# debbiemarkslab/BEAR

Measured on AMD Instinct MI355X. Metric: k-mer contexts/sec (DM-marginal+grad h), k=13, higher is better.
Workload: dtype f64

## Files before the change

### bear_amd/csrc/kernels_plan.h

```cpp
#pragma once
#include "kernels_sorted.h"

#ifndef PLN_THREADS
#define PLN_THREADS 1024
#endif
#define PLN_WAVES (PLN_THREADS / 64)
#ifndef PLN_UNITS
#define PLN_UNITS 32
#endif
#define PLN_NI (PLN_UNITS * 64)
#ifndef PLN_NI_CUT
#define PLN_NI_CUT PLN_NI
#endif
#ifndef PLN_RMAX
#define PLN_RMAX 1664
#endif
#ifndef PLN_HCAP
#define PLN_HCAP 128
#endif
#define PLN_NBIG 4096
#define PLN_BLOCKS_PER_CU (1024 / PLN_THREADS)
#define PLN_QUAD 4
#define PLN_LIVE_STRIDE (PLN_RMAX + 8)
#define PLN_SENTINEL (PLN_RMAX * 5)
#ifndef PLN_NBUF
#define PLN_NBUF 2
#endif
#define PLN_BLOCK_MAX (64 + PLN_RMAX + PLN_NI * 2 + PLN_HCAP * (2 + 4 + 2 + 8))

struct pln_tile {
  uint64_t row0;
  uint32_t rows_items;
  uint32_t off16;
  uint32_t hc_hr;
  uint32_t blk16;
  uint64_t pad;
};
static_assert(sizeof(pln_tile) == 32, "tile descriptors are fetched with one s_load_dwordx8");
#ifndef PLN_CHUNK
#define PLN_CHUNK 128
#endif
#ifndef PLN_DMA_WAVES
#define PLN_DMA_WAVES 2
#endif
#ifndef PLN_PREFETCH_KIB
#define PLN_PREFETCH_KIB 24
#endif
#define PLN_DESC_CHUNK 32
#define PLN_DESC_PAD (2 * PLN_DESC_CHUNK)

struct pln_layout {
  uint32_t nrow, items, hoff, hcnt, hrow, hn, end;
};
__host__ __device__ inline pln_layout pln_block_layout(uint32_t rows, uint32_t n_light, uint32_t hc, uint32_t hr) {
  pln_layout L;
  L.nrow = 64u;
  L.items = L.nrow + ((rows + 15u) & ~15u);
  L.hoff = L.items + (((n_light + 63u) & ~63u) * 2u);
  L.hcnt = L.hoff + (((hc + 7u) & ~7u) * 2u);
  L.hrow = L.hcnt + (((hc + 3u) & ~3u) * 4u);
  L.hn = L.hrow + (((hr + 7u) & ~7u) * 2u);
  L.end = L.hn + (((hr + 1u) & ~1u) * 8u);
  return L;
}

struct pln_heavy_col {
  uint64_t off;
  uint64_t c;
};

struct pln_heavy_row {
  uint64_t row;
  double n;
};

__global__ __launch_bounds__(256) void plan_scan_kernel(const uint32_t *__restrict__ counts, uint64_t n_rows, int ncol,
                                                        uint8_t *__restrict__ quad_light,
                                                        unsigned long long *__restrict__ heavy_counts,
                                                        unsigned long long *__restrict__ hist) {
  __shared__ uint32_t s_heavy[3];
  __shared__ uint32_t s_hist[2 * SRT_NKEY];
  __shared__ uint32_t s_big[PLN_NBIG + 1];
  __shared__ unsigned long long s_total, s_cells;
  __shared__ uint32_t s_cmax;
  unsigned long long my_total = 0ull;
  uint32_t my_cells = 0u, my_cmax = 0u;
  if (threadIdx.x == 0) {
    s_total = s_cells = 0ull;
    s_cmax = 0u;
  }
  if (threadIdx.x < 3) s_heavy[threadIdx.x] = 0;
  if (threadIdx.x < 2 * SRT_NKEY) s_hist[threadIdx.x] = 0;
  for (uint32_t k = threadIdx.x; k <= PLN_NBIG; k += 256) s_big[k] = 0;
  __syncthreads();
  const uint64_t n_quads = (n_rows + PLN_QUAD - 1) / PLN_QUAD;
  for (uint64_t g = (uint64_t)blockIdx.x * 256 + threadIdx.x; g < n_quads; g += (uint64_t)gridDim.x * 256) {
    uint32_t light = 0, qhc = 0, qhr = 0;
    for (uint64_t r = PLN_QUAD * g; r < PLN_QUAD * g + PLN_QUAD && r < n_rows; ++r) {
      uint32_t nsat = 0, hcol = 0;
#pragma unroll
      for (int b = 0; b < 5; ++b) {
        const uint32_t c = counts[r * 5 + b];
        const uint32_t s = nsat + c;
        nsat = s < nsat ? 0xffffffffu : s;
        my_total += c;
        my_cells += c != 0u;
        my_cmax = c > my_cmax ? c : my_cmax;
        if (b < ncol) {
          light += (c != 0 && c <= SRT_CL);
          hcol += (c > SRT_CL);
        }
      }
      qhc += hcol;
      qhr += nsat > SRT_CL;
      if (hcol) atomicAdd(&s_heavy[0], hcol);
      if (nsat > SRT_CL) {
        atomicAdd(&s_heavy[1], 1u);
        if (nsat <= PLN_NBIG) atomicAdd(&s_big[nsat], 1u);
      } else if (nsat != 0) atomicAdd(&s_hist[nsat - 1], 1u);
      const uint32_t c4 = counts[r * 5 + 4];
      if (ncol == 4 && c4 > SRT_CL) atomicAdd(&s_heavy[2], 1u);
      else if (ncol == 4 && c4 != 0) atomicAdd(&s_hist[SRT_NKEY + c4 - 1], 1u);
    }
    quad_light[g] = (uint8_t)light;
    quad_light[n_quads + g] = (uint8_t)qhc;
    quad_light[2 * n_quads + g] = (uint8_t)qhr;
  }
  if (my_total) {
    atomicAdd(&s_total, my_total);
    atomicAdd(&s_cells, (unsigned long long)my_cells);
    atomicMax(&s_cmax, my_cmax);
  }
  __syncthreads();
  if (threadIdx.x == 0 && s_total) {
    atomicAdd(&heavy_counts[6], s_total);
    atomicAdd(&heavy_counts[7], s_cells);
    atomicMax(&heavy_counts[8], (unsigned long long)s_cmax);
  }
  if (threadIdx.x < 3 && s_heavy[threadIdx.x]) atomicAdd(&heavy_counts[threadIdx.x], (unsigned long long)s_heavy[threadIdx.x]);
  if (threadIdx.x < 2 * SRT_NKEY && s_hist[threadIdx.x]) atomicAdd(&hist[threadIdx.x], (unsigned long long)s_hist[threadIdx.x]);
  for (uint32_t k = threadIdx.x; k <= PLN_NBIG; k += 256)
    if (s_big[k]) atomicAdd(&hist[2 * SRT_NKEY + k], (unsigned long long)s_big[k]);
}

#define PLN_CUT_CHUNK_MAX 8192
static inline uint32_t plan_cut_chunk(uint64_t n_quads) { return n_quads <= 50000000ull ? 2048u : (uint32_t)PLN_CUT_CHUNK_MAX; }
#define PLN_CUT_SPAN (PLN_RMAX / PLN_QUAD)

__device__ __forceinline__ uint64_t plan_cut_one(const uint8_t *__restrict__ quad, uint64_t n_quads, uint64_t q0, uint32_t *items,
                                                 uint32_t *hcol, uint32_t *hrow) {
  uint32_t it = 0, hc = 0, hr = 0, rows = 0;
  uint64_t q = q0;
  while (q < n_quads && rows + PLN_QUAD <= PLN_RMAX && it + quad[q] <= PLN_NI_CUT) {
    it += quad[q];
    if (hcol) {
      hc += quad[n_quads + q];
      hr += quad[2 * n_quads + q];
    }
    rows += PLN_QUAD;
    ++q;
  }
  *items = it;
  if (hcol) {
    *hcol = hc;
    *hrow = hr;
  }
  return q;
}
__global__ __launch_bounds__(256) void plan_cut_step_kernel(const uint8_t *__restrict__ quad, uint64_t n_quads, uint64_t n_chunks,
                                                            uint32_t chunk, uint16_t *__restrict__ step) {
  const uint64_t k = (uint64_t)blockIdx.x * 256 + threadIdx.x;
  if (k >= n_chunks) return;
  const uint64_t q0 = k * chunk, q_end = q0 + chunk < n_quads ? q0 + chunk : n_quads;
  uint64_t r = q0;
  uint32_t items = 0;
  for (uint64_t q = q0; q < q_end; ++q) {
    if (r < q) {
      r = q;
      items = 0;
    }
    while (r < n_quads && (uint32_t)(r - q + 1) * PLN_QUAD <= PLN_RMAX && items + quad[r] <= PLN_NI_CUT) items += quad[r++];
    step[q] = (uint16_t)(r - q);
    items -= quad[q];
  }
}
__global__ __launch_bounds__(256) void plan_cut_walk_kernel(const uint16_t *__restrict__ step, uint64_t n_quads, uint64_t n_chunks,
                                                            uint32_t chunk, uint32_t *__restrict__ walk) {
  const uint64_t id = (uint64_t)blockIdx.x * 256 + threadIdx.x;
  if (id >= n_chunks * PLN_CUT_SPAN) return;
  const uint64_t k = id / PLN_CUT_SPAN, j = id - k * PLN_CUT_SPAN, end = (k + 1) * chunk;
  uint64_t q = k * chunk + j;
  uint32_t cnt = 0;
  while (q < end && q < n_quads) {
    q += step[q];
    ++cnt;
  }
  walk[id] = (uint32_t)(q >= end ? q - end : 0) | (cnt << 16);
}
static_assert(PLN_CUT_CHUNK_MAX < 65536 && PLN_CUT_SPAN < 65536 && PLN_CUT_SPAN <= 2048, "walk table: 16-bit fields; a tile is shorter than a chunk");
// ... 226 lines not shown
    if (tid == 31) E[31] = (uint16_t)hr_cap;
#pragma unroll
    for (int k = 0; k < RPT; ++k)
#pragma unroll
      for (int b = 0; b < 5; ++b)
        if (c[k][b] != 0) sorted[offs[(c[k][b] - 1) * SRT_REP + rep] + rank[k][b]] = (uint16_t)((tid + 1024u * k) * 5 + b);
    __syncthreads();
#ifdef BEAR_DET_BUILD
    {
      for (uint32_t i = tid; i < PLN_NI; i += 1024) {
        uint32_t key = 0;
        for (uint32_t q = 1; q < SRT_CL; ++q) key += offs[q * SRT_REP] <= i ? 1u : 0u;
        comp[i] = i < n_light ? (key << 16) | sorted[i] : 0xffffffffu;
      }
      __syncthreads();
      for (uint32_t size = 2; size <= PLN_NI; size <<= 1)
        for (uint32_t stride = size >> 1; stride > 0; stride >>= 1) {
          const uint32_t lo = 2u * tid - (tid & (stride - 1u)), hi = lo + stride;
          if (tid < PLN_NI / 2) {
            const bool up = (lo & size) == 0u;
            const uint32_t a = comp[lo], bq = comp[hi];
            if ((a > bq) == up) {
              comp[lo] = bq;
              comp[hi] = a;
            }
          }
          __syncthreads();
        }
      for (uint32_t i = tid; i < n_light; i += 1024) sorted[i] = (uint16_t)(comp[i] & 0xffffu);
      __syncthreads();
      const uint32_t nhc = s_hc < hc_cap ? s_hc : hc_cap, nhr = s_hr < hr_cap ? s_hr : hr_cap;
      if (tid < nhc) hkey[tid] = ((unsigned long long)hoff[tid] << 32) | hcnt[tid];
      __syncthreads();
      if (tid < nhc) {
        uint32_t r = 0;
        for (uint32_t q = 0; q < nhc; ++q) r += hkey[q] < hkey[tid] ? 1u : 0u;
        htmp[r] = hkey[tid];
      }
      __syncthreads();
      if (tid < nhc) {
        hoff[tid] = (uint16_t)(htmp[tid] >> 32);
        hcnt[tid] = (uint32_t)htmp[tid];
      }
      __syncthreads();
      if (tid < nhr) hkey[tid] = ((unsigned long long)hrow[tid] << 48) | tid;
      if (tid < nhr) htmp[tid] = (unsigned long long)__double_as_longlong(hn[tid]);
      __syncthreads();
      uint32_t r = 0;
      unsigned long long mine = 0ull, myn = 0ull;
      if (tid < nhr) {
        for (uint32_t q = 0; q < nhr; ++q) r += hkey[q] < hkey[tid] ? 1u : 0u;
        mine = hkey[tid];
        myn = htmp[tid];
      }
      __syncthreads();
      if (tid < nhr) {
        hrow[r] = (uint16_t)(mine >> 48);
        hn[r] = __longlong_as_double((long long)myn);
      }
      __syncthreads();
    }
#endif
    const uint32_t padded = (n_light + 63u) & ~63u;
    for (uint32_t i = tid; i < padded; i += 1024) items[i] = i < n_light ? sorted[i] : (uint16_t)PLN_SENTINEL;
    __syncthreads();
  }
}

__global__ __launch_bounds__(1024) void plan_live_kernel(const pln_tile *__restrict__ tiles, uint64_t n_tiles,
                                                         const unsigned char *__restrict__ stream, uint16_t *__restrict__ live) {
  constexpr int RPT = (PLN_RMAX + 1023) / 1024;
  __shared__ uint32_t cnt[RPT * 16];
  const uint32_t tid = threadIdx.x, lane = tid & 63, wave = tid >> 6;
  for (uint64_t t = blockIdx.x; t < n_tiles; t += gridDim.x) {
    const pln_tile ti = tiles[t];
    const uint32_t rows = ti.rows_items >> 16;
    const uint8_t *nrow = stream + (size_t)ti.off16 * 16 + 64;
    uint16_t *out = live + t * PLN_LIVE_STRIDE;
    unsigned long long mask[RPT];
#pragma unroll
    for (int k = 0; k < RPT; ++k) {
      const uint32_t lr = tid + 1024u * k;
      mask[k] = __builtin_amdgcn_ballot_w64(lr < rows && nrow[lr] != 0);
      if (lane == 0) cnt[k * 16 + wave] = (uint32_t)__builtin_popcountll(mask[k]);
    }
    __syncthreads();
    uint32_t total = 0;
#pragma unroll
    for (int k = 0; k < RPT; ++k) {
      uint32_t base = total;
      for (int w = 0; w < 16; ++w) {
        const uint32_t c = cnt[k * 16 + w];
        if (w < (int)wave) base += c;
        total += c;
      }
      if ((mask[k] >> lane) & 1ull) out[1 + base + (uint32_t)__builtin_popcountll(mask[k] & ((1ull << lane) - 1ull))] = (uint16_t)(tid + 1024u * k);
    }
    if (tid == 0) out[0] = (uint16_t)total;
    __syncthreads();
  }
}

struct pln_view {
  const pln_tile *tiles;
  const unsigned char *stream;
  const pln_heavy_col *heavy_col;
  const pln_heavy_row *heavy_row;
  const uint64_t *heavy_stop;
  const unsigned long long *hist;
  const unsigned long long *hist_big;
  int big_in_hist;
  uint64_t n_tiles, n_heavy_col, n_heavy_row, n_heavy_stop;
  const uint16_t *live;
  const uint16_t *live2;
  int subset;
};

__device__ __forceinline__ void pln_big_totals(const pln_view &pv, double A, double scale, uint64_t gtid, uint64_t gsz, const double2 *logtab,
                                               double &acc_D, double &acc_P) {
  if (!pv.hist_big) return;
  for (uint64_t n = SRT_CL + 1 + gtid; n <= PLN_NBIG; n += gsz) {
    const unsigned long long m = pv.hist_big[n];
    if (m) {
      const bear_dp o = srt_general_fast(A, (double)n, logtab);
      acc_D -= (double)m * o.D;
      acc_P = __builtin_fma(scale * (double)m, o.P, acc_P);
    }
  }
}
__device__ __forceinline__ bool pln_in_big_hist(const pln_view &pv, double n) { return pv.big_in_hist && n <= (double)PLN_NBIG; }

__device__ __forceinline__ uint32_t pln_dma(void *lds, const void *src, uint32_t bytes, uint32_t wave, uint32_t lane,
                                            uint32_t first) {
  const uint32_t d = (uint32_t)(uintptr_t)lds;
  const unsigned char *s = static_cast<const unsigned char *>(src) + lane * 16u;
  const uint32_t pieces = (bytes + 1023u) >> 10;
  uint32_t issued = 0;
  for (uint32_t piece = (wave + PLN_WAVES - (first % PLN_WAVES)) % PLN_WAVES; piece < pieces; piece += PLN_WAVES) {
    const unsigned char *g = s + (piece << 10);
    const uint32_t m = srt_uniform(d + (piece << 10));
    if ((piece << 10) + lane * 16u < bytes)
      {
      uint32_t keep_m0;
      asm volatile("s_mov_b32 %0, m0\n\ts_mov_b32 m0, %2\n\ts_nop 0\n\tglobal_load_lds_dwordx4 %1, off\n\ts_mov_b32 m0, %0"
                   : "=&s"(keep_m0)
                   : "v"(g), "s"(m)
                   : "memory");
    }
    ++issued;
  }
  return issued;
}

__device__ __forceinline__ void pln_dma_piece(void *lds, const void *src, uint32_t bytes, uint32_t piece, uint32_t lane) {
  const uint32_t m = srt_uniform((uint32_t)(uintptr_t)lds + (piece << 10));
  const unsigned char *g = static_cast<const unsigned char *>(src) + (piece << 10) + lane * 16u;
  if ((piece << 10) + lane * 16u < bytes)
    {
      uint32_t keep_m0;
      asm volatile("s_mov_b32 %0, m0\n\ts_mov_b32 m0, %2\n\ts_nop 0\n\tglobal_load_lds_dwordx4 %1, off\n\ts_mov_b32 m0, %0"
                   : "=&s"(keep_m0)
                   : "v"(g), "s"(m)
                   : "memory");
    }
}

__device__ __forceinline__ void pln_wait_all_but(uint32_t younger) {
  switch (younger) {
    case 0: asm volatile("s_waitcnt vmcnt(0)" ::: "memory"); break;
    case 1: asm volatile("s_waitcnt vmcnt(1)" ::: "memory"); break;
    case 2: asm volatile("s_waitcnt vmcnt(2)" ::: "memory"); break;
    case 3: asm volatile("s_waitcnt vmcnt(3)" ::: "memory"); break;
    case 4: asm volatile("s_waitcnt vmcnt(4)" ::: "memory"); break;
    case 5: asm volatile("s_waitcnt vmcnt(5)" ::: "memory"); break;
    case 6: asm volatile("s_waitcnt vmcnt(6)" ::: "memory"); break;
    case 7: asm volatile("s_waitcnt vmcnt(7)" ::: "memory"); break;
    case 8: asm volatile("s_waitcnt vmcnt(8)" ::: "memory"); break;
    default: asm volatile("s_waitcnt vmcnt(0)" ::: "memory"); break;
  }
}

__device__ __forceinline__ pln_tile pln_load_tile(const pln_view &pv, uint64_t t) {
  pln_tile ti;
  ti.row0 = 0;
  ti.rows_items = 0;
  ti.off16 = 0;
  ti.hc_hr = 0;
  ti.blk16 = 0;
  ti.pad = 0;
  if (t < pv.n_tiles) {
    const __attribute__((address_space(4))) pln_tile *tc = (const __attribute__((address_space(4))) pln_tile *)(uintptr_t)pv.tiles;
    ti.row0 = tc[t].row0;
    ti.rows_items = tc[t].rows_items;
    ti.off16 = tc[t].off16;
    ti.hc_hr = tc[t].hc_hr;
    ti.blk16 = tc[t].blk16;
    ti.pad = tc[t].pad;
  }
  return ti;
}

__device__ __forceinline__ uint32_t pln_ticket(uint32_t *counter, uint32_t lane) {
  uint32_t t = 0;
  if (lane == 0)
    asm volatile("ds_add_rtn_u32 %0, %1, %2\n\ts_waitcnt lgkmcnt(0)" : "=&v"(t) : "v"((uint32_t)(uintptr_t)counter), "v"(1u) : "memory");
  return srt_uniform(t);
}

#ifdef BEAR_DET_BUILD
#define PLN_FOR_UNITS(w, counter, n, first, stride) for (uint32_t w = (first); w < (n); w += (stride))
#else
#define PLN_FOR_UNITS(w, counter, n, first, stride) for (uint32_t w = pln_ticket(counter, lane); w < (n); w = pln_ticket(counter, lane))
#endif
#if defined(BEAR_DET_BUILD) || defined(PLN_NO_FIRST_UNIT_DEALT)
#define PLN_FOR_UNITS_F(w, counter, n, first, stride) PLN_FOR_UNITS(w, counter, n, first, stride)
#define PLN_TICKET_START(stride) 0u
#else
#define PLN_FOR_UNITS_F(w, counter, n, first, stride) for (uint32_t w = (first); w < (n); w = pln_ticket(counter, lane))
#define PLN_TICKET_START(stride) ((uint32_t)(stride))
#endif

__device__ __forceinline__ uint32_t pln_ticket_issue(uint32_t *counter, uint32_t lane) {
  uint32_t t = 0;
  if (lane == 0) t = atomicAdd(counter, 1u);
  return t;
}

__device__ __forceinline__ uint32_t pln_unit_counts(const uint16_t *E, uint32_t n_light, uint32_t un, uint32_t lane,
                                                    uint32_t *cmin, uint32_t *cmax) {
  const uint32_t base = un * 64u, idx = base + lane;
  const uint32_t last = (base + 64u <= n_light ? base + 64u : n_light) - 1u;
  const uint32_t e = lane < 30u ? (uint32_t)E[lane] : 0xffffffffu;
  uint32_t lo, hi;
  asm("s_bcnt1_i32_b64 %0, %1" : "=s"(lo) : "s"(__builtin_amdgcn_ballot_w64(e <= base)) : "scc");
  asm("s_bcnt1_i32_b64 %0, %1" : "=s"(hi) : "s"(__builtin_amdgcn_ballot_w64(e <= last)) : "scc");
  uint32_t c = lo;
  for (uint32_t k = lo; k < hi; ++k) c += idx >= (uint32_t)__builtin_amdgcn_readlane((int)e, (int)k) ? 1u : 0u;
  *cmin = base + 64u <= n_light ? lo : 0u;
  *cmax = hi;
  return idx < n_light ? c : 0u;
}

struct pln_buf_n {
  double pri[PLN_RMAX * 5 + 2];
  __attribute__((aligned(16))) unsigned char blk[PLN_BLOCK_MAX];
};
struct pln_lds_n {
  pln_buf_n buf[PLN_NBUF];
  double2 logtab[BEAR_LOGTAB_N];
  double tabD[SRT_NKEY];
  double tabP[SRT_NKEY];
  uint32_t ticket[PLN_NBUF];
  __attribute__((aligned(16))) pln_tile desc[2][PLN_DESC_CHUNK];
  __attribute__((aligned(16))) uint32_t pf_scratch[64];
};

__device__ __forceinline__ pln_tile pln_desc(const pln_tile (*ring)[PLN_DESC_CHUNK], uint64_t j, uint64_t count) {
  pln_tile ti;
  ti.row0 = 0;
  ti.rows_items = 0;
  ti.off16 = 0;
  ti.hc_hr = 0;
  ti.blk16 = 0;
  ti.pad = 0;
  if (j < count) {
    const uint32_t *d = reinterpret_cast<const uint32_t *>(&ring[(j >> 5) & 1u][j & 31u]);
    const uint32_t lo = srt_uniform(d[0]), hi = srt_uniform(d[1]);
    ti.row0 = ((uint64_t)hi << 32) | lo;
    ti.rows_items = srt_uniform(d[2]);
    ti.off16 = srt_uniform(d[3]);
    ti.hc_hr = srt_uniform(d[4]);
    ti.blk16 = srt_uniform(d[5]);
  }
  return ti;
}

template <bool NORM, bool AR>
__global__ __launch_bounds__(PLN_THREADS, 4) void dm_prior_plan_kernel(const double *__restrict__ prior,
                                                                                    uint64_t n_rows, bear_params prm_arg,
                                                                                    pln_view pv,
                                                                                    const double2 *__restrict__ logtab_g,
                                                                                    double *__restrict__ partials,
                                                                                    const bear_step_io io
#ifdef PLN_STAMPS
                                                                                    , unsigned long long *__restrict__ dbg
#endif
                                                                                    ) {
  extern __shared__ __attribute__((aligned(16))) unsigned char srt_smem[];
  pln_lds_n &S = *reinterpret_cast<pln_lds_n *>(srt_smem);
  const bear_params prm = bear_params_of(prm_arg, io);
  const uint32_t tid = threadIdx.x, lane = tid & 63, wave = srt_uniform(tid >> 6);
  const double u = prm.inv_h, eps = prm.eps, eps5 = 5.0 * prm.eps;
  double acc[2] = {0.0, 0.0};

  if (tid < BEAR_LOGTAB_N) S.logtab[tid] = logtab_g[tid];
  if (tid < SRT_NKEY) {
    const bear_dp o = srt_general_fast(u + eps5, (double)(tid + 1), logtab_g);
    S.tabD[tid] = o.D;
    S.tabP[tid] = o.P;
  }
  if (tid < PLN_NBUF) {
    S.buf[tid].pri[PLN_SENTINEL] = 1.0;
    S.ticket[tid] = PLN_TICKET_START(PLN_WAVES - PLN_DMA_WAVES);
  }

  const bool dma_wave = wave >= PLN_WAVES - PLN_DMA_WAVES;
  const uint32_t dw = wave - (PLN_WAVES - PLN_DMA_WAVES);
  auto stage = [&](const pln_tile &ti, uint32_t b) {
    const uint32_t rows = ti.rows_items >> 16;
    if (rows == 0) return;
    const uint32_t pbytes = (rows * 40u) & ~15u, bbytes = ti.blk16 * 16u;
    const unsigned char *psrc = reinterpret_cast<const unsigned char *>(prior + ti.row0 * 5);
    const unsigned char *bsrc = pv.stream + (size_t)ti.off16 * 16;
    for (uint32_t pc = dw; (pc << 10) < bbytes; pc += PLN_DMA_WAVES) pln_dma_piece(S.buf[b].blk, bsrc, bbytes, pc, lane);
    for (uint32_t pc = dw; (pc << 10) < pbytes; pc += PLN_DMA_WAVES) pln_dma_piece(S.buf[b].pri, psrc, pbytes, pc, lane);
    if (dw == 0 && ((rows * 40u) & 15u)) {
      const __attribute__((address_space(4))) double *tail =
          (const __attribute__((address_space(4))) double *)(uintptr_t)(prior + (ti.row0 + rows) * 5 - 1);
      const double v = *tail;
      if (lane == 0) S.buf[b].pri[rows * 5 - 1] = v;
    }
  };

  constexpr uint32_t PF_INSTR = (NORM || AR) ? PLN_PREFETCH_KIB / 8u : 0u;
  auto prefetch_behind = [&](const pln_tile &ti) -> uint32_t {
    const uint32_t rows = ti.rows_items >> 16;
    if (PF_INSTR == 0 || rows == 0) return 0u;
    const uint64_t end_bytes = n_rows * 40ull, base = (ti.row0 + rows) * 40ull;
    const uint32_t m = srt_uniform((uint32_t)(uintptr_t)S.pf_scratch);
    uint32_t issued = 0;
    for (uint32_t k = dw; k < PF_INSTR; k += PLN_DMA_WAVES) {
      uint64_t off = base + ((uint64_t)(k * 64u + lane) << 7);
      if (off + 4u > end_bytes) off = end_bytes - 4u;
      const unsigned char *g = reinterpret_cast<const unsigned char *>(prior) + off;
      uint32_t keep_m0;
      asm volatile("s_mov_b32 %0, m0\n\ts_mov_b32 m0, %2\n\ts_nop 0\n\tglobal_load_lds_dword %1, off\n\ts_mov_b32 m0, %0"
                   : "=&s"(keep_m0)
                   : "v"(g), "s"(m)
                   : "memory");
      ++issued;
    }
    return issued;
  };
  uint32_t pf_young = 0;
#ifdef PLN_STAMPS
  unsigned long long tph[8] = {0, 0, 0, 0, 0, 0, 0, 0}, t_prev = __builtin_amdgcn_s_memtime();
  int prev_kind = 0;
#define PLN_STAMP(k)                                              \
  {                                                               \
    const unsigned long long now = __builtin_amdgcn_s_memtime();  \
    tph[k] += now - t_prev;                                       \
    t_prev = now;                                                 \
  }
#else
#define PLN_STAMP(k)
#endif
  static_assert(PLN_NBUF == 2, "the DMA-wave protocol below is written for a two-slot ring");
  const uint64_t G = gridDim.x;
  const uint64_t first = (pv.n_tiles * (uint64_t)blockIdx.x) / G, count = (pv.n_tiles * ((uint64_t)blockIdx.x + 1)) / G - first;
  auto fetch_desc = [&](uint64_t j0) {
    if (dw == 0 && j0 < count)
      pln_dma_piece(S.desc[(j0 >> 5) & 1u], pv.tiles + first + j0, PLN_DESC_CHUNK * (uint32_t)sizeof(pln_tile), 0u, lane);
  };
  if (dma_wave) {
    __builtin_amdgcn_s_setprio(3);
    fetch_desc(0);
    fetch_desc(PLN_DESC_CHUNK);
    srt_wait_dma();
  }
  __syncthreads();
  pln_tile cur = pln_desc(S.desc, 0, count), nxt = pln_desc(S.desc, 1, count);
  if (dma_wave) stage(cur, 0);
  uint32_t slot = 0;
  for (uint64_t j = 0; j < count; ++j) {
#ifdef PLN_STAMPS
    PLN_STAMP(prev_kind)
    prev_kind = 4;
#endif
    if (dma_wave) pln_wait_all_but(pf_young);
    PLN_STAMP(1)
    srt_sync();
    PLN_STAMP(2)
    const pln_tile nn = pln_desc(S.desc, j + 2, count);
    if (dma_wave) {
      if ((j & (PLN_DESC_CHUNK - 1)) == 0 && j != 0) fetch_desc(j + PLN_DESC_CHUNK);
      stage(nxt, slot ^ 1u);
      pf_young = prefetch_behind(nxt);
      cur = nxt;
      nxt = nn;
      slot ^= 1u;
      continue;
    }
    PLN_STAMP(3)

    const pln_buf_n &B = S.buf[slot];
    const uint32_t rows = cur.rows_items >> 16, n_light = cur.rows_items & 0xffffu;
    const uint32_t hc = cur.hc_hr >> 16, hr = cur.hc_hr & 0xffffu;
    const pln_layout L = pln_block_layout(rows, n_light, hc, hr);
    const uint16_t *E = reinterpret_cast<const uint16_t *>(B.blk);
    const uint8_t *nrow = B.blk + L.nrow;
    const uint16_t *items = reinterpret_cast<const uint16_t *>(B.blk + L.items);
    if (tid == 0) S.ticket[(slot + 1) % PLN_NBUF] = PLN_TICKET_START(PLN_WAVES - PLN_DMA_WAVES);
    const uint32_t n_hcu = (hc + 63u) >> 6, n_hru = AR ? 0u : (hr + 63u) >> 6, n_heavy = n_hcu + n_hru;
    const uint32_t n_units = (n_light + 63u) >> 6;
    const uint32_t n_work = n_heavy + n_units + ((NORM || AR) ? 0u : (rows + PLN_CHUNK - 1u) / PLN_CHUNK);
    PLN_FOR_UNITS_F(w, &S.ticket[slot], n_work, wave, PLN_WAVES - PLN_DMA_WAVES) {
#ifdef PLN_STAMPS
      {
        const unsigned long long now = __builtin_amdgcn_s_memtime();
        tph[prev_kind] += now - t_prev;
        t_prev = now;
        prev_kind = w < n_heavy ? 5 : (w < n_heavy + n_units ? 6 : 7);
      }
#endif
      if (w < n_hcu) {
        const uint32_t i = w * 64u + lane;
        if (i < hc) {
          const uint32_t off = reinterpret_cast<const uint16_t *>(B.blk + L.hoff)[i];
          const double cnt = (double)reinterpret_cast<const uint32_t *>(B.blk + L.hcnt)[i];
          if (AR) {
            acc[0] = __builtin_fma(cnt, bear_log_tab(B.pri[off] + eps, S.logtab), acc[0]);
          } else {
            const double x = __builtin_fma(B.pri[off], u, eps);
            const bear_dp o = srt_general_fast(x, cnt, S.logtab);
            acc[0] += o.D;
            acc[1] = __builtin_fma(eps - x, o.P, acc[1]);
          }
        }
        continue;
      }
      if (w < n_heavy) {
        const uint32_t i = (w - n_hcu) * 64u + lane;
        if (i < hr) {
          const double *f = &B.pri[(uint32_t)reinterpret_cast<const uint16_t *>(B.blk + L.hrow)[i] * 5u];
          const double A = NORM ? u + eps5 : __builtin_fma(((f[0] + f[1]) + (f[2] + f[3])) + f[4], u, eps5);
          const bear_dp o = srt_general_fast(A, reinterpret_cast<const double *>(B.blk + L.hn)[i], S.logtab);
          acc[0] -= o.D;
          acc[1] = __builtin_fma(A - eps5, o.P, acc[1]);
        }
        continue;
      }
      if (NORM || AR || w < n_heavy + n_units) {
        const uint32_t un = n_heavy + n_units - 1u - w;
        uint32_t cmin, cmax;
        const uint32_t ci[1] = {pln_unit_counts(E, n_light, un, lane, &cmin, &cmax)};
        const uint32_t off = items[un * 64u + lane];
        if (AR) {
          acc[0] = __builtin_fma((double)ci[0], bear_log_tab(B.pri[off] + eps, S.logtab), acc[0]);
          continue;
        }
        const double x[1] = {__builtin_fma(B.pri[off], u, eps)};
        bear_dp o[1];
        srt_light<1>(x, ci, cmin, cmax, S.logtab, o);
        acc[0] += o[0].D;
        acc[1] = __builtin_fma(eps - x[0], o[0].P, acc[1]);
        continue;
      }
      static_assert(PLN_CHUNK == 128, "two adjacent contexts per lane");
      const uint32_t row0c = (w - n_heavy - n_units) * PLN_CHUNK + 2u * lane;
      double S5[2];
      uint32_t nn_[2];
      {
        const uint32_t rr = row0c < rows ? row0c : 0u;
        const double2 *src = reinterpret_cast<const double2 *>(&B.pri[rr * 5]);
        const double2 v0 = src[0], v1 = src[1], v2 = src[2], v3 = src[3], v4 = src[4];
        S5[0] = ((v0.x + v0.y) + (v1.x + v1.y)) + v2.x;
        S5[1] = ((v2.y + v3.x) + (v3.y + v4.x)) + v4.y;
#pragma unroll
        for (int q = 0; q < 2; ++q) {
          const uint32_t n = row0c + q < rows ? (uint32_t)nrow[rr + q] : 0u;
          nn_[q] = n == 255u ? 0u : n;
        }
      }
#pragma unroll
      for (int q = 0; q < PLN_CHUNK / 64; ++q) {
        const uint32_t n = nn_[q];
        const bool shared = __builtin_fabs(S5[q] - 1.0) <= SRT_SUM1_TOL;
        if (n != 0 && shared) {
          acc[0] -= S.tabD[n - 1];
          acc[1] = __builtin_fma(u, S.tabP[n - 1], acc[1]);
        }
        const uint32_t own = (n != 0 && !shared) ? n : 0u;
        if (__builtin_amdgcn_ballot_w64(own != 0)) {
          uint32_t cm = own;
#pragma unroll
          for (int off = 32; off > 0; off >>= 1) {
            const uint32_t o2 = (uint32_t)__shfl_xor((int)cm, off, 64);
            cm = o2 > cm ? o2 : cm;
          }
          const double xa[1] = {own ? __builtin_fma(S5[q], u, eps5) : 1.0};
          const uint32_t ca[1] = {own};
          bear_dp o[1];
          srt_light<1>(xa, ca, 0u, srt_uniform(cm), S.logtab, o);
          acc[0] -= o[0].D;
          acc[1] = __builtin_fma(xa[0] - eps5, o[0].P, acc[1]);
        }
      }
    }
    cur = nxt;
    nxt = nn;
    slot ^= 1u;
  }
  srt_wait_dma();
#ifdef PLN_STAMPS
  if (lane == 0 && dbg) {
    for (int k = 0; k < 8; ++k) dbg[((size_t)blockIdx.x * PLN_WAVES + wave) * 8 + k] = tph[k];
  }
#endif
  const uint64_t gtid = (uint64_t)blockIdx.x * PLN_THREADS + tid, gsz = (uint64_t)gridDim.x * PLN_THREADS;
  for (uint64_t i = gtid; i < pv.n_heavy_col; i += gsz) {
    const pln_heavy_col h = pv.heavy_col[i];
    if (AR) {
      acc[0] = __builtin_fma((double)h.c, bear_log_tab(prior[h.off] + eps, S.logtab), acc[0]);
      continue;
    }
    const double x = __builtin_fma(prior[h.off], u, eps);
    const bear_dp o = srt_general_fast(x, (double)h.c, S.logtab);
    acc[0] += o.D;
    acc[1] = __builtin_fma(eps - x, o.P, acc[1]);
  }
  for (uint64_t i = gtid; !AR && i < pv.n_heavy_row; i += gsz) {
    const pln_heavy_row h = pv.heavy_row[i];
    const double *f = prior + h.row * 5;
    const double A = __builtin_fma(((f[0] + f[1]) + (f[2] + f[3])) + f[4], u, eps5);
    const bear_dp o = srt_general_fast(A, h.n, S.logtab);
    acc[0] -= o.D;
    acc[1] = __builtin_fma(A - eps5, o.P, acc[1]);
  }
  if (NORM && !AR && blockIdx.x == 0 && tid < SRT_CL) {
    const double m = (double)pv.hist[tid];
    acc[0] -= m * S.tabD[tid];
    acc[1] = __builtin_fma(u * m, S.tabP[tid], acc[1]);
  }
  __syncthreads();
  block_finish<2>(acc, partials, io);
}

struct pln_buf_r {
  uint32_t ref[PLN_RMAX * 5 + 4];
  __attribute__((aligned(16))) unsigned char blk[PLN_BLOCK_MAX];
};
#define PLN_RSLOT 3
struct pln_lds_r {
  pln_buf_r buf[PLN_RSLOT];
  double2 logtab[BEAR_LOGTAB_N];
  double tabD[2][SRT_NKEY];
  double tabP[2][SRT_NKEY];
  uint32_t meta[PLN_RSLOT][2];
  uint32_t ticket[PLN_RSLOT];
  uint32_t landed[PLN_RSLOT];
  uint32_t left[PLN_RSLOT];
};
__device__ __forceinline__ uint32_t pln_peek(const uint32_t *p) {
  return srt_uniform(__hip_atomic_load(p, __ATOMIC_RELAXED, __HIP_MEMORY_SCOPE_WORKGROUP));
}

template <bool AR>
__global__ __launch_bounds__(PLN_THREADS, 4) void dm_ref_plan_kernel(const uint32_t *__restrict__ ref,
                                                                                  uint64_t n_rows, bear_params prm_arg,
                                                                                  pln_view pv,
                                                                                  const double2 *__restrict__ logtab_g,
                                                                                  double *__restrict__ partials,
                                                                                  const bear_step_io io, const bear_apply_io apply) {
  extern __shared__ __attribute__((aligned(16))) unsigned char srt_smem[];
  pln_lds_r &S = *reinterpret_cast<pln_lds_r *>(srt_smem);
  const bear_params prm = bear_params_of(prm_arg, io);
  const uint32_t tid = threadIdx.x, lane = tid & 63, wave = srt_uniform(tid >> 6);
  const double u = prm.inv_h, eps = prm.eps;
  const double A = u + 5.0 * eps;
  const double x4 = prm.nw * prm.V * u + eps;
  const double VU = prm.V * u;
  const double tau = prm.tau;
  const double w2c = tau * (eps + 0.25 * VU);
  const double nwV = prm.nw * prm.V;
  double acc[4] = {0.0, 0.0, 0.0, 0.0};

  if (tid < BEAR_LOGTAB_N) S.logtab[tid] = logtab_g[tid];
  if (tid < 2 * SRT_NKEY) {
    const int which = tid / SRT_NKEY, j = tid % SRT_NKEY;
    const bear_dp o = srt_general_fast(which ? x4 : A, (double)(j + 1), logtab_g);
    S.tabD[which][j] = o.D;
    S.tabP[which][j] = o.P;
  }
  if (tid < PLN_RSLOT) {
    S.landed[tid] = S.left[tid] = 0u;
    S.ticket[tid] = PLN_TICKET_START(PLN_WAVES - PLN_DMA_WAVES);
  }
  if (tid < 4 * PLN_RSLOT) S.buf[tid >> 2].ref[PLN_SENTINEL + (tid & 3)] = 0;

  const bool dma_wave = wave >= PLN_WAVES - PLN_DMA_WAVES;
  const uint32_t dw = wave - (PLN_WAVES - PLN_DMA_WAVES);
  constexpr uint32_t CWAVES = PLN_WAVES - PLN_DMA_WAVES;
  auto stage = [&](const pln_tile &ti, uint32_t b) {
    const uint32_t rows = ti.rows_items >> 16;
    const uint32_t rbytes = rows * 20u, rb16 = rbytes & ~15u, bbytes = ti.blk16 * 16u;
    const unsigned char *rsrc = reinterpret_cast<const unsigned char *>(ref + ti.row0 * 5);
    const unsigned char *bsrc = pv.stream + (size_t)ti.off16 * 16;
    for (uint32_t pc = 0; (pc << 10) < bbytes; ++pc) pln_dma_piece(S.buf[b].blk, bsrc, bbytes, pc, lane);
    for (uint32_t pc = 0; (pc << 10) < rb16; ++pc) pln_dma_piece(S.buf[b].ref, rsrc, rb16, pc, lane);
    if (rbytes & 15u) {
      const uint32_t w0 = rb16 >> 2, nw = (rbytes & 15u) >> 2;
      const __attribute__((address_space(4))) uint32_t *tail =
          (const __attribute__((address_space(4))) uint32_t *)(uintptr_t)(ref + ti.row0 * 5 + w0);
      const uint32_t v0 = tail[0], v1 = nw > 1 ? tail[1] : 0u, v2 = nw > 2 ? tail[2] : 0u;
      if (lane == 0) {
        S.buf[b].ref[w0] = v0;
        if (nw > 1) S.buf[b].ref[w0 + 1] = v1;
        if (nw > 2) S.buf[b].ref[w0 + 2] = v2;
      }
    }
    if (lane == 0) {
      S.meta[b][0] = ti.rows_items;
      S.meta[b][1] = ti.hc_hr;
      S.ticket[b] = PLN_TICKET_START(PLN_WAVES - PLN_DMA_WAVES);
    }
  };
  auto alpha_from = [&](double rb, double R) {
    const double dev = __builtin_fma(rb + eps, bear_rcp(R), -0.25);
    return __builtin_fma(__builtin_fma(prm.E, dev, 0.25), VU, eps);
  };
  auto accumulate = [&](double x, const bear_dp &o) {
    const double w1 = eps - x;
    acc[0] += o.D;
    acc[1] = __builtin_fma(w1, o.P, acc[1]);
    acc[2] = __builtin_fma(__builtin_fma(-tau, x, w2c), o.P, acc[2]);
    acc[3] = __builtin_fma(nwV * w1, o.P, acc[3]);
  };
  auto accumulate_ar = [&](double rb, double R, double c) {
    const double dev = __builtin_fma(rb + eps, bear_rcp(R), -0.25);
    const double f = __builtin_fma(prm.E, dev, 0.25) * prm.V;
    const double p = f + eps;
    const double dLdf = c * bear_rcp(p);
    acc[0] = __builtin_fma(c, bear_log_tab(p, S.logtab), acc[0]);
    acc[2] = __builtin_fma(dLdf, -prm.tauE * dev * prm.V, acc[2]);
    acc[3] = __builtin_fma(dLdf, -nwV * f, acc[3]);
  };

  const uint64_t G = gridDim.x;
  const uint64_t first = (pv.n_tiles * (uint64_t)blockIdx.x) / G, count = (pv.n_tiles * ((uint64_t)blockIdx.x + 1)) / G - first;
  __syncthreads();
  if (dma_wave) {
    __builtin_amdgcn_s_setprio(3);
    pln_tile ti = pln_load_tile(pv, dw < count ? first + dw : pv.n_tiles);
    for (uint64_t j = dw; j < count; j += PLN_DMA_WAVES) {
      const uint32_t b = (uint32_t)(j % PLN_RSLOT), gen = (uint32_t)(j / PLN_RSLOT);
      const pln_tile ti_next = pln_load_tile(pv, j + PLN_DMA_WAVES < count ? first + j + PLN_DMA_WAVES : pv.n_tiles);
      while (pln_peek(&S.left[b]) < CWAVES * gen) __builtin_amdgcn_s_sleep(1);
      stage(ti, b);
      srt_wait_dma();
      asm volatile("s_waitcnt lgkmcnt(0)" ::: "memory");
      if (lane == 0) atomicAdd(&S.landed[b], 1u);
      ti = ti_next;
    }
  }
  for (uint64_t j = 0; !dma_wave && j < count; ++j) {
    const uint32_t slot = (uint32_t)(j % PLN_RSLOT), gen = (uint32_t)(j / PLN_RSLOT);
    while (pln_peek(&S.landed[slot]) < gen + 1u) __builtin_amdgcn_s_sleep(1);
    const pln_buf_r &B = S.buf[slot];
    const uint32_t rows_items = srt_uniform(S.meta[slot][0]), hc_hr = srt_uniform(S.meta[slot][1]);
    const uint32_t rows = rows_items >> 16, n_light = rows_items & 0xffffu;
    const uint32_t hc = hc_hr >> 16;
    const pln_layout L = pln_block_layout(rows, n_light, hc, hc_hr & 0xffffu);
    const uint16_t *E = reinterpret_cast<const uint16_t *>(B.blk);
    const uint16_t *items = reinterpret_cast<const uint16_t *>(B.blk + L.items);
    const uint32_t n_hcu = (hc + 63u) >> 6;
    const uint32_t n_units = (n_light + 63u) >> 6;
    PLN_FOR_UNITS_F(w, &S.ticket[slot], n_hcu + n_units, wave, CWAVES) {
      if (w < n_hcu) {
        const uint32_t i = w * 64u + lane;
        if (i < hc) {
          const uint32_t off = reinterpret_cast<const uint16_t *>(B.blk + L.hoff)[i];
          const uint32_t *rr = &B.ref[((off * 52429u) >> 18) * 5u];
          const double R = (double)(((uint64_t)rr[0] + rr[1]) + ((uint64_t)rr[2] + rr[3])) + 4.0 * eps;
          const double cnt = (double)reinterpret_cast<const uint32_t *>(B.blk + L.hcnt)[i];
          if (AR) {
            accumulate_ar((double)B.ref[off], R, cnt);
          } else {
            const double x = alpha_from((double)B.ref[off], R);
            accumulate(x, srt_general_fast(x, cnt, S.logtab));
          }
        }
        continue;
// ... 437 lines not shown
```

Measured before the change: 131.7 billion.

## Fold row-count terms into histogram and fetch nrow bytes only on sum failures

For the general (non-normalised) mode, the per-row shared-prior term now comes from the global count histogram, as the normalised mode already does. Each tile only checks whether its prior rows sum to one and runs the per-row correction for rows that do not. The nrow section of the block stream is no longer DMA'd by default. When a tile has sum failures, nrow is read from global memory, and the tile's next reuse of that buffer stages nrow again. The change also turns on prefetch-behind for this mode and adds an optional nontemporal DMA flag, which means more complexity and a chance of extra global reads on non-normalised inputs.

```diff
diff --git a/bear_amd/csrc/kernels_plan.h b/bear_amd/csrc/kernels_plan.h
--- a/bear_amd/csrc/kernels_plan.h
+++ b/bear_amd/csrc/kernels_plan.h
@@ -45,6 +45,15 @@
 #endif
 #ifndef PLN_PREFETCH_KIB
 #define PLN_PREFETCH_KIB 24
+#endif
+#ifndef PLN_GEN_PREFETCH
+#define PLN_GEN_PREFETCH 1
+#endif
+#ifndef PLN_GEN_NT
+#define PLN_GEN_NT 0
+#endif
+#ifndef PLN_GEN_NROW_ON_DEMAND
+#define PLN_GEN_NROW_ON_DEMAND 1
 #endif
 #define PLN_DESC_CHUNK 32
 #define PLN_DESC_PAD (2 * PLN_DESC_CHUNK)
@@ -577,16 +586,23 @@
   return issued;
 }
 
+template <bool NT = false>
 __device__ __forceinline__ void pln_dma_piece(void *lds, const void *src, uint32_t bytes, uint32_t piece, uint32_t lane) {
   const uint32_t m = srt_uniform((uint32_t)(uintptr_t)lds + (piece << 10));
   const unsigned char *g = static_cast<const unsigned char *>(src) + (piece << 10) + lane * 16u;
   if ((piece << 10) + lane * 16u < bytes)
     {
       uint32_t keep_m0;
-      asm volatile("s_mov_b32 %0, m0\n\ts_mov_b32 m0, %2\n\ts_nop 0\n\tglobal_load_lds_dwordx4 %1, off\n\ts_mov_b32 m0, %0"
-                   : "=&s"(keep_m0)
-                   : "v"(g), "s"(m)
-                   : "memory");
+      if (NT)
+        asm volatile("s_mov_b32 %0, m0\n\ts_mov_b32 m0, %2\n\ts_nop 0\n\tglobal_load_lds_dwordx4 %1, off nt\n\ts_mov_b32 m0, %0"
+                     : "=&s"(keep_m0)
+                     : "v"(g), "s"(m)
+                     : "memory");
+      else
+        asm volatile("s_mov_b32 %0, m0\n\ts_mov_b32 m0, %2\n\ts_nop 0\n\tglobal_load_lds_dwordx4 %1, off\n\ts_mov_b32 m0, %0"
+                     : "=&s"(keep_m0)
+                     : "v"(g), "s"(m)
+                     : "memory");
     }
 }
 
@@ -676,9 +692,12 @@
   double tabD[SRT_NKEY];
   double tabP[SRT_NKEY];
   uint32_t ticket[PLN_NBUF];
+  uint32_t sum_fail[PLN_NBUF];
+  uint32_t nrow_in[PLN_NBUF];
   __attribute__((aligned(16))) pln_tile desc[2][PLN_DESC_CHUNK];
   __attribute__((aligned(16))) uint32_t pf_scratch[64];
 };
+static_assert(sizeof(pln_lds_n) <= 160 * 1024, "one block per CU: the planned mode-N kernels' LDS");
 
 __device__ __forceinline__ pln_tile pln_desc(const pln_tile (*ring)[PLN_DESC_CHUNK], uint64_t j, uint64_t count) {
   pln_tile ti;
@@ -727,18 +746,29 @@
   if (tid < PLN_NBUF) {
     S.buf[tid].pri[PLN_SENTINEL] = 1.0;
     S.ticket[tid] = PLN_TICKET_START(PLN_WAVES - PLN_DMA_WAVES);
+    S.sum_fail[tid] = 0xffffffffu;
   }
 
   const bool dma_wave = wave >= PLN_WAVES - PLN_DMA_WAVES;
   const uint32_t dw = wave - (PLN_WAVES - PLN_DMA_WAVES);
-  auto stage = [&](const pln_tile &ti, uint32_t b) {
+  constexpr bool GEN = !NORM && !AR;
+  constexpr bool NT = GEN && PLN_GEN_NT;
+  auto stage = [&](const pln_tile &ti, uint32_t b, bool with_nrow) {
     const uint32_t rows = ti.rows_items >> 16;
     if (rows == 0) return;
     const uint32_t pbytes = (rows * 40u) & ~15u, bbytes = ti.blk16 * 16u;
     const unsigned char *psrc = reinterpret_cast<const unsigned char *>(prior + ti.row0 * 5);
     const unsigned char *bsrc = pv.stream + (size_t)ti.off16 * 16;
-    for (uint32_t pc = dw; (pc << 10) < bbytes; pc += PLN_DMA_WAVES) pln_dma_piece(S.buf[b].blk, bsrc, bbytes, pc, lane);
-    for (uint32_t pc = dw; (pc << 10) < pbytes; pc += PLN_DMA_WAVES) pln_dma_piece(S.buf[b].pri, psrc, pbytes, pc, lane);
+    if (GEN && dw == 0 && lane == 0) S.nrow_in[b] = with_nrow ? 1u : 0u;
+    if (!GEN || with_nrow) {
+      for (uint32_t pc = dw; (pc << 10) < bbytes; pc += PLN_DMA_WAVES) pln_dma_piece<NT>(S.buf[b].blk, bsrc, bbytes, pc, lane);
+    } else {
+      const uint32_t items0 = pln_block_layout(rows, ti.rows_items & 0xffffu, ti.hc_hr >> 16, ti.hc_hr & 0xffffu).items;
+      if (dw == PLN_DMA_WAVES - 1) pln_dma_piece<NT>(S.buf[b].blk, bsrc, 64u, 0u, lane);
+      for (uint32_t pc = dw; (pc << 10) < bbytes - items0; pc += PLN_DMA_WAVES)
+        pln_dma_piece<NT>(S.buf[b].blk + items0, bsrc + items0, bbytes - items0, pc, lane);
+    }
+    for (uint32_t pc = dw; (pc << 10) < pbytes; pc += PLN_DMA_WAVES) pln_dma_piece<NT>(S.buf[b].pri, psrc, pbytes, pc, lane);
     if (dw == 0 && ((rows * 40u) & 15u)) {
       const __attribute__((address_space(4))) double *tail =
           (const __attribute__((address_space(4))) double *)(uintptr_t)(prior + (ti.row0 + rows) * 5 - 1);
@@ -747,7 +777,7 @@
     }
   };
 
-  constexpr uint32_t PF_INSTR = (NORM || AR) ? PLN_PREFETCH_KIB / 8u : 0u;
+  constexpr uint32_t PF_INSTR = (NORM || AR || PLN_GEN_PREFETCH) ? PLN_PREFETCH_KIB / 8u : 0u;
   auto prefetch_behind = [&](const pln_tile &ti) -> uint32_t {
     const uint32_t rows = ti.rows_items >> 16;
     if (PF_INSTR == 0 || rows == 0) return 0u;
@@ -795,7 +825,7 @@
   }
   __syncthreads();
   pln_tile cur = pln_desc(S.desc, 0, count), nxt = pln_desc(S.desc, 1, count);
-  if (dma_wave) stage(cur, 0);
+  if (dma_wave) stage(cur, 0, !PLN_GEN_NROW_ON_DEMAND);
   uint32_t slot = 0;
   for (uint64_t j = 0; j < count; ++j) {
 #ifdef PLN_STAMPS
@@ -809,7 +839,7 @@
     const pln_tile nn = pln_desc(S.desc, j + 2, count);
     if (dma_wave) {
       if ((j & (PLN_DESC_CHUNK - 1)) == 0 && j != 0) fetch_desc(j + PLN_DESC_CHUNK);
-      stage(nxt, slot ^ 1u);
+      stage(nxt, slot ^ 1u, !GEN || !PLN_GEN_NROW_ON_DEMAND || srt_uniform(S.sum_fail[slot ^ 1u]) == (uint32_t)j);
       pf_young = prefetch_behind(nxt);
       cur = nxt;
       nxt = nn;
@@ -828,14 +858,57 @@
     if (tid == 0) S.ticket[(slot + 1) % PLN_NBUF] = PLN_TICKET_START(PLN_WAVES - PLN_DMA_WAVES);
     const uint32_t n_hcu = (hc + 63u) >> 6, n_hru = AR ? 0u : (hr + 63u) >> 6, n_heavy = n_hcu + n_hru;
     const uint32_t n_units = (n_light + 63u) >> 6;
-    const uint32_t n_work = n_heavy + n_units + ((NORM || AR) ? 0u : (rows + PLN_CHUNK - 1u) / PLN_CHUNK);
+    const uint32_t n_work = n_heavy + n_units;
+    static_assert(PLN_CHUNK == 128, "two adjacent contexts per lane");
+    for (uint32_t c = wave; GEN && c * PLN_CHUNK < rows; c += PLN_WAVES - PLN_DMA_WAVES) {
+      const uint32_t row0c = c * PLN_CHUNK + 2u * lane;
+      const uint32_t rr = row0c < rows ? row0c : 0u;
+      const double2 *src = reinterpret_cast<const double2 *>(&B.pri[rr * 5]);
+      const double2 v0 = src[0], v1 = src[1], v2 = src[2], v3 = src[3], v4 = src[4];
+      const double S5[2] = {((v0.x + v0.y) + (v1.x + v1.y)) + v2.x, ((v2.y + v3.x) + (v3.y + v4.x)) + v4.y};
+      bool bad[2];
+#pragma unroll
+      for (int q = 0; q < 2; ++q) bad[q] = row0c + q < rows && !(__builtin_fabs(S5[q] - 1.0) <= SRT_SUM1_TOL);
+      if (__builtin_amdgcn_ballot_w64(bad[0] || bad[1])) {
+        if (lane == 0) S.sum_fail[slot] = (uint32_t)(j + 1);
+        uint32_t nn_[2];
+        if (!PLN_GEN_NROW_ON_DEMAND || srt_uniform(S.nrow_in[slot])) {
+#pragma unroll
+          for (int q = 0; q < 2; ++q) nn_[q] = bad[q] ? (uint32_t)nrow[rr + q] : 0u;
+        } else {
+          const uint8_t *g = pv.stream + (size_t)cur.off16 * 16 + L.nrow;
+#pragma unroll
+          for (int q = 0; q < 2; ++q) nn_[q] = bad[q] ? (uint32_t)g[rr + q] : 0u;
+        }
+#pragma unroll
+        for (int q = 0; q < PLN_CHUNK / 64; ++q) {
+          const uint32_t own = nn_[q] == 255u ? 0u : nn_[q];
+          if (__builtin_amdgcn_ballot_w64(own != 0)) {
+            uint32_t cm = own;
+#pragma unroll
+            for (int off = 32; off > 0; off >>= 1) {
+              const uint32_t o2 = (uint32_t)__shfl_xor((int)cm, off, 64);
+              cm = o2 > cm ? o2 : cm;
+            }
+            const double xa[1] = {own ? __builtin_fma(S5[q], u, eps5) : 1.0};
+            const uint32_t ca[1] = {own};
+            bear_dp o[1];
+            srt_light<1>(xa, ca, 0u, srt_uniform(cm), S.logtab, o);
+            if (own) {
+              acc[0] += S.tabD[own - 1] - o[0].D;
+              acc[1] = __builtin_fma(xa[0] - eps5, o[0].P, __builtin_fma(-u, S.tabP[own - 1], acc[1]));
+            }
+          }
+        }
+      }
+    }
     PLN_FOR_UNITS_F(w, &S.ticket[slot], n_work, wave, PLN_WAVES - PLN_DMA_WAVES) {
 #ifdef PLN_STAMPS
       {
         const unsigned long long now = __builtin_amdgcn_s_memtime();
         tph[prev_kind] += now - t_prev;
         t_prev = now;
-        prev_kind = w < n_heavy ? 5 : (w < n_heavy + n_units ? 6 : 7);
+        prev_kind = w < n_heavy ? 5 : 6;
       }
 #endif
       if (w < n_hcu) {
@@ -865,7 +938,7 @@
         }
         continue;
       }
-      if (NORM || AR || w < n_heavy + n_units) {
+      {
         const uint32_t un = n_heavy + n_units - 1u - w;
         uint32_t cmin, cmax;
         const uint32_t ci[1] = {pln_unit_counts(E, n_light, un, lane, &cmin, &cmax)};
@@ -881,46 +954,6 @@
         acc[1] = __builtin_fma(eps - x[0], o[0].P, acc[1]);
         continue;
       }
-      static_assert(PLN_CHUNK == 128, "two adjacent contexts per lane");
-      const uint32_t row0c = (w - n_heavy - n_units) * PLN_CHUNK + 2u * lane;
-      double S5[2];
-      uint32_t nn_[2];
-      {
-        const uint32_t rr = row0c < rows ? row0c : 0u;
-        const double2 *src = reinterpret_cast<const double2 *>(&B.pri[rr * 5]);
-        const double2 v0 = src[0], v1 = src[1], v2 = src[2], v3 = src[3], v4 = src[4];
-        S5[0] = ((v0.x + v0.y) + (v1.x + v1.y)) + v2.x;
-        S5[1] = ((v2.y + v3.x) + (v3.y + v4.x)) + v4.y;
-#pragma unroll
-        for (int q = 0; q < 2; ++q) {
-          const uint32_t n = row0c + q < rows ? (uint32_t)nrow[rr + q] : 0u;
-          nn_[q] = n == 255u ? 0u : n;
-        }
-      }
-#pragma unroll
-      for (int q = 0; q < PLN_CHUNK / 64; ++q) {
-        const uint32_t n = nn_[q];
-        const bool shared = __builtin_fabs(S5[q] - 1.0) <= SRT_SUM1_TOL;
-        if (n != 0 && shared) {
-          acc[0] -= S.tabD[n - 1];
-          acc[1] = __builtin_fma(u, S.tabP[n - 1], acc[1]);
-        }
-        const uint32_t own = (n != 0 && !shared) ? n : 0u;
-        if (__builtin_amdgcn_ballot_w64(own != 0)) {
-          uint32_t cm = own;
-#pragma unroll
-          for (int off = 32; off > 0; off >>= 1) {
-            const uint32_t o2 = (uint32_t)__shfl_xor((int)cm, off, 64);
-            cm = o2 > cm ? o2 : cm;
-          }
-          const double xa[1] = {own ? __builtin_fma(S5[q], u, eps5) : 1.0};
-          const uint32_t ca[1] = {own};
-          bear_dp o[1];
-          srt_light<1>(xa, ca, 0u, srt_uniform(cm), S.logtab, o);
-          acc[0] -= o[0].D;
-          acc[1] = __builtin_fma(xa[0] - eps5, o[0].P, acc[1]);
-        }
-      }
     }
     cur = nxt;
     nxt = nn;
@@ -952,7 +985,7 @@
     acc[0] -= o.D;
     acc[1] = __builtin_fma(A - eps5, o.P, acc[1]);
   }
-  if (NORM && !AR && blockIdx.x == 0 && tid < SRT_CL) {
+  if (!AR && blockIdx.x == 0 && tid < SRT_CL) {
     const double m = (double)pv.hist[tid];
     acc[0] -= m * S.tabD[tid];
     acc[1] = __builtin_fma(u * m, S.tabP[tid], acc[1]);
```

Result: faster. 136.0 billion, median of 6 (+3.3%).
